# shivendrra/shredword

Measured on AMD Instinct MI355X. Metric: encoded MB/s (input bytes) + Mtokens/s at 32k merges, 1/2/4/8 MI355X vs CPU ref, higher is better.
Workload: dtype int32

## Files before the change

shredword_amd/csrc/encode.hip:

```cpp
#include <hip/hip_runtime.h>

#include <algorithm>
#include <cstdio>
#include <cstring>
#include <string>
#include <vector>

#include "encoder.h"
#include "kernels.h"
#include "long_split.h"
#include "pairtable.h"
#include "presplit_kernel.h"
#include "split_classify.h"
#include "specials_find.h"
#include "test_options.h"

using namespace sw;

static thread_local std::string g_err;
int32_t sw::set_error(int32_t code, const std::string& msg) {
  g_err = msg;
  return code;
}

// ... 559 lines not shown
    }
    SpFind f;
    f.bytes = d_bytes; f.n_bytes = n_bytes; f.str_off = d_str_off; f.n_str = n_str;
    f.tile_slo = h->ws.d_tile_slo; f.n_tiles = n_tiles;
    f.cbits = h->d_spf; f.chosen = h->d_spf + 64 * n_tiles;
    f.tcand = h->d_spf + 128 * n_tiles; f.tcnt = f.tcand + n_tiles;
    f.flag = (unsigned int*)(f.tcnt + n_tiles);
    f.list = h->d_spf_list; f.tcap = tcap;
    int64_t* toff = h->d_spf_off;
    int64_t* toff2 = h->d_spf_off + n_tiles + n_parts;
    int64_t* total2 = toff2 + n_tiles + n_parts;
    const dim3 gw((unsigned)((n_tiles + kWaves - 1) / kWaves)), bw(kThreads);
    HIP_TRY(hipMemsetAsync(f.flag, 0, sizeof(unsigned int), st));
    hipLaunchKernelGGL(k_tile_strings, dim3((unsigned)((n_tiles + 255) / 256)), dim3(256), 0, st, d_str_off, n_str,
                       n_tiles, h->ws.d_tile_slo, nullptr);
    const bool swar = h->spt.n_first <= kSpMaxFirstSwar;
    const size_t lds_tab = sizeof(uint32_t) * (size_t)h->spt.img_words;
    if (swar) hipLaunchKernelGGL(k_sp_find<true>, gw, bw, lds_tab, st, h->spt, f);
    else hipLaunchKernelGGL(k_sp_find<false>, gw, bw, lds_tab, st, h->spt, f);
    HIP_TRY(launch_scan(st, f.tcnt, n_tiles, toff + n_tiles, toff, d_count));
    const dim3 ge((unsigned)((n_tiles + kWaves * kSfEmitTiles - 1) / (kWaves * kSfEmitTiles)));
    hipLaunchKernelGGL(k_sp_emit, ge, bw, 0, st, h->spt, f, (const int64_t*)toff, d_pos, d_len, d_id);
    const dim3 gg(std::min<unsigned>(gw.x, kSfGlobalBlocks));
    if (swar) hipLaunchKernelGGL(k_sp_detect<true>, gg, bw, 0, st, h->spt, f);
    else hipLaunchKernelGGL(k_sp_detect<false>, gg, bw, 0, st, h->spt, f);
    hipLaunchKernelGGL(k_sp_resolve, gg, bw, lds_tab, st, h->spt, f);
    hipLaunchKernelGGL(k_sp_count, gg, bw, 0, st, f);
    HIP_TRY(launch_scan(st, f.tcnt, n_tiles, toff2 + n_tiles, toff2, total2));
    hipLaunchKernelGGL(k_sp_write, gg, bw, 0, st, h->spt, f, (const int64_t*)toff2, d_pos, d_len, d_id);
    hipLaunchKernelGGL(k_sp_fix_count, dim3(1), dim3(64), 0, st, (const unsigned int*)f.flag, (const int64_t*)total2,
                       d_count);
    HIP_TRY(hipGetLastError());
  }
  HIP_TRY(hipEventRecord(h->ws_done, st));
  h->ws_stream = st;
  h->ws_pending = true;
  return SW_OK;
}

namespace {

EncArgs make_args(sw_encoder* h, const uint8_t* d_bytes, int64_t n_bytes, const int64_t* d_str_off, int64_t n_str,
                  const uint64_t* d_chunk_bits, const SpArgs& spa, int64_t* d_out_off, int64_t n_tiles) {
  Workspace& w = h->ws;
  EncArgs a;
  a.bytes = d_bytes; a.n_bytes = n_bytes; a.bits = d_chunk_bits; a.n_words = (n_bytes + 63) / 64;
  a.str_off = d_str_off; a.n_str = n_str; a.table = h->table; a.chunks = h->chunks;
  a.scratch = w.d_scratch; a.res = w.d_res;
  a.tile_slots = w.d_tile_slots; a.tile_nref = w.d_tile_nref; a.rlist = w.d_rlist; a.tile_cnt = w.d_tile_cnt;
  a.dtab = w.d_dtab; a.dedupe = h->dedupe ? 1u : 0u; a.dfp_mask = h->dedupe_fp_mask;
  {
    const uint32_t lmask = (uint32_t)(launch_dd_slots(h, n_bytes) - 1);
    a.dmask = h->dedupe_slots ? std::min<uint32_t>(lmask, (uint32_t)(h->dedupe_slots - 1)) : lmask;
  }
  a.dexact = h->dedupe_exact ? (uint32_t)kDdExactMax : 0u;
  a.dres = w.d_dres;
  a.dcnt = w.d_dcnt;
  a.dd_full = w.d_ddfull;
  a.llist = w.d_llist; a.l_count = w.d_lcount;
  a.big_count = w.d_big; a.big_list = w.d_big + 1;
  a.out_off = d_out_off; a.tile_slo = w.d_tile_slo;
  a.n_tiles = n_tiles; a.qtmp = w.d_res; a.bcnt = w.d_bcnt; a.boff = w.d_boff; a.q_total = w.d_qtotal;
  a.queue = w.d_queue; a.stamps = w.d_stamps;
  a.inv = h->d_inv; a.n_inv = h->n_inv; a.ids16 = h->ids16 ? 1u : 0u;
  a.lstart = w.lp.wstart; a.llen = w.lp.wlen; a.n_long = &w.lp.ctl[kLcWave]; a.lcap = w.lp.lcap;
  a.sp = spa;
  const unsigned long long prev_merges = h->h_ddfull ? __atomic_load_n(&h->h_ddfull[2], __ATOMIC_RELAXED) : 0ULL;
  a.staged_heads = (h->staged_heads == 1 || (h->staged_heads == 0 && h->dedupe && prev_merges > kStagedMinMerges)) ? 1u : 0u;
  return a;
}

template <bool kSp>
hipError_t launch_classify_pair(sw_encoder* h, hipStream_t st, const EncArgs& a, const PbArgs* pg, int pattern,
                                hipEvent_t c0, hipEvent_t c1) {
  const dim3 gc((unsigned)((a.n_tiles + kWaves - 1) / kWaves)), gr(kRedoGrid), b(kThreads);
  unsigned int* count = h->ws.d_redo;
  int64_t* tiles = (int64_t*)(count + 2);
  hipError_t e = c0 ? hipEventRecord(c0, st) : hipSuccess;
  if (e != hipSuccess) return e;
  if (pg) {
    const RedoList redo{count, tiles};
    const uint32_t* edge = h->ws.d_edge;
    uint32_t* pbits = (uint32_t*)h->ws.d_pbits.get();
    hipLaunchKernelGGL(k_split_classify<kSp>, gc, b, 0, st, a, *pg, pattern, edge, pbits, redo);
    if (c1 && (e = hipEventRecord(c1, st)) != hipSuccess) return e;
    hipLaunchKernelGGL(k_split_redo<kSp>, gr, b, 0, st, a, *pg, pattern, edge, pbits, redo);
  } else {
    hipLaunchKernelGGL(k_classify<kSp>, gc, b, 0, st, a, count, tiles);
    if (c1 && (e = hipEventRecord(c1, st)) != hipSuccess) return e;
    hipLaunchKernelGGL(k_classify_big<kSp>, gr, b, 0, st, a, (const unsigned int*)count, (const int64_t*)tiles);
  }
  return hipGetLastError();
}

int32_t launch_classify(sw_encoder* h, hipStream_t st, const EncArgs& a, int32_t pattern, bool fused) {
  const int64_t n_tiles = a.n_tiles;
  const size_t dtab_bytes = sizeof(uint64_t) * kDdWords * ((size_t)a.dmask + 1);
  const int64_t edge_threads = (n_tiles + 1 + 255) / 256 * 256;
  const bool clr_in_edges = fused && dtab_bytes % 16 == 0 && (int64_t)(dtab_bytes / 16) <= 16 * edge_threads;
  if (h->dedupe && !clr_in_edges) HIP_TRY(hipMemsetAsync(h->ws.d_dtab, 0, dtab_bytes, st));
  hipEvent_t c0 = nullptr, c1 = nullptr;
  if (h->timing) HIP_TRY(h->ev_cls.next(&c0, &c1));
  const PbArgs pg{a.bytes, a.n_bytes, a.str_off, a.n_str, a.tile_slo, a.sp};
  if (fused)
    hipLaunchKernelGGL(k_edges, dim3((unsigned)((n_tiles + 1 + 255) / 256)), dim3(256), 0, st, pg, n_tiles, (int)pattern,
                       h->ws.d_edge.get(), h->ws.d_redo.get(), h->dedupe && clr_in_edges ? (uint4*)h->ws.d_dtab.get() : nullptr,
                       (int64_t)(dtab_bytes / 16));
  else
    HIP_TRY(hipMemsetAsync(h->ws.d_redo, 0, sizeof(unsigned int), st));
  HIP_TRY(a.sp.n > 0 ? launch_classify_pair<true>(h, st, a, fused ? &pg : nullptr, (int)pattern, c0, c1)
                     : launch_classify_pair<false>(h, st, a, fused ? &pg : nullptr, (int)pattern, c0, c1));
  if (c1) ++h->ev_cls.used;
  return SW_OK;
}

template <bool kWide, bool k16, bool kWF>
void launch_merge_buckets(const EncArgs& a, const hipStream_t (&ms)[4]) {
  const dim3 pg(2048), pb(kThreads);
  hipLaunchKernelGGL((k_merge_bucket<kWide, k16, 32, kWF>), pg, pb, 0, ms[0], a, 8, 9);
  hipLaunchKernelGGL((k_merge_bucket<kWide, k16, 16, kWF>), pg, pb, 0, ms[1], a, 5, 7);
  hipLaunchKernelGGL((k_merge_bucket<kWide, k16, 8, kWF>), pg, pb, 0, ms[2], a, 3, 4);
  hipLaunchKernelGGL((k_merge_bucket<kWide, k16, 4, kWF>), pg, pb, 0, ms[1], a, 0, 2);
}

template <bool kWide, bool k16, bool kWF>
int32_t launch_merges_as(sw_encoder* h, hipStream_t st, const EncArgs& a) {
  const int64_t n_tiles = a.n_tiles;
  const bool split = h->split_ok && h->long_split;
  hipStream_t ms[4] = {st, st, st, st};
  if (h->merge_fork) {
    for (int k = 0; k < 2; ++k) {
      HIP_TRY(h->s_fork[k].ensure());
      HIP_TRY(h->ev_join[k].ensure());
    }
    HIP_TRY(h->ev_fork.ensure());
    HIP_TRY(h->ev_fork_long.ensure());
    HIP_TRY(hipEventRecord(h->ev_fork_long, st));
    HIP_TRY(hipStreamWaitEvent(h->s_fork[1], h->ev_fork_long, 0));
    ms[1] = h->s_fork[0];
    ms[3] = h->s_fork[1];
  }
  HIP_TRY((launch_long<kWide, k16>(h, ms[3], a, split, 1)));
  HIP_TRY(launch_scan(st, h->ws.d_bcnt, kNumBuckets * n_tiles, h->ws.d_part, h->ws.d_boff, h->ws.d_qtotal));
  hipLaunchKernelGGL(k_scatter, dim3((unsigned)((n_tiles + 15) / 16)), dim3(kThreads), 0, st, a);
  if (h->merge_fork) {
    HIP_TRY(hipEventRecord(h->ev_fork, st));
    for (int k = 0; k < 2; ++k) HIP_TRY(hipStreamWaitEvent(h->s_fork[k], h->ev_fork, 0));
  }
  HIP_TRY((launch_long<kWide, k16>(h, ms[3], a, split, 2)));
  launch_merge_buckets<kWide, k16, kWF>(a, ms);
  if (h->merge_fork) {
    for (int k = 0; k < 2; ++k) {
      HIP_TRY(hipEventRecord(h->ev_join[k], h->s_fork[k]));
      HIP_TRY(hipStreamWaitEvent(st, h->ev_join[k], 0));
    }
  }
  HIP_TRY(hipGetLastError());
  return SW_OK;
}

int32_t launch_merges(sw_encoder* h, hipStream_t st, const EncArgs& a) {
  if (h->table.wide) return launch_merges_as<true, false, false>(h, st, a);
  if (h->ids16 && h->split_ok) return launch_merges_as<false, true, true>(h, st, a);
  if (h->ids16) return launch_merges_as<false, true, false>(h, st, a);
  return launch_merges_as<false, false, false>(h, st, a);
}

// ... 190 lines not shown
```

shredword_amd/csrc/kernels.h:

```cpp
#pragma once
#include <hip/hip_runtime.h>

#include <cstdint>
#include <type_traits>

#include "args.h"
#include "chunktable.h"
#include "table.h"

namespace sw {

constexpr int kThreads = 256;
constexpr int kWaves = kThreads / 64;
__device__ __forceinline__ int wave_in_block() {
  return (int)(threadIdx.x >> 6);
}
__device__ __forceinline__ int64_t tile_end(int64_t t0, int64_t n_bytes) {
  return (int64_t)min((int32_t)t0 + (int32_t)kTile, (int32_t)n_bytes);
}
__device__ __forceinline__ int wave_in_block_s() {
  return __builtin_amdgcn_readfirstlane((int)(threadIdx.x >> 6));
}
constexpr int kShort = 32;
constexpr int kWin = kTile + 64;
// ... 602 lines not shown
      if (prev_taken) M &= ~1ULL;
      uint64_t T = M;
      if (p0 == p1) {
        const uint64_t E = 0x5555555555555555ULL;
        const uint64_t S = M & ~(M << 1);
        const uint64_t runs_even = M & ~(M + (S & E));
        T = (runs_even & E) | (M & ~runs_even & ~E);
      }
      const uint64_t consumed = (T << 1) | (prev_taken ? 1ULL : 0ULL);
      const uint64_t keep = __ballot(valid) & ~consumed;
      const bool take = (T >> lane) & 1ULL;
      const bool next_take = lane < 63 ? ((T >> (lane + 1)) & 1ULL) : true;
      const int64_t pos = w + __popcll(keep & lt_mask);
      wave_sync_mem();
      if ((keep >> lane) & 1ULL) {
        id[pos] = take ? nv : e;
        rk[pos] = (take || next_take) ? RECOMP : er;
      }
      w += __popcll(keep);
      prev_taken = (T >> 63) & 1ULL;
    }
    n = w;
    wave_sync_mem();
  }
  return n;
}

struct SpArgs {
  const int64_t* pos;
  const int32_t* len;
  const int32_t* id;
  int64_t n;
  const int64_t* tile_sp;
  const int64_t* tile_spw;
};

struct EncArgs {
  const uint8_t* bytes;
  int64_t n_bytes;
  const uint64_t* bits;
  int64_t n_words;
  const int64_t* str_off;
  int64_t n_str;
  DevTable table;
  DevChunkTable chunks;
  int32_t* scratch;
  uint32_t* res;
  uint32_t* tile_cnt;
  uint32_t* tile_slots;
  uint32_t* tile_nref;
  uint32_t* rlist;
  int64_t* out_off;
  const int64_t* tile_slo;
  int64_t n_tiles;
  uint32_t* qtmp;
  uint32_t* bcnt;
  const int64_t* boff;
  const int64_t* q_total;
  uint64_t* queue;
  uint64_t* dtab;
  uint32_t dmask;
  uint32_t dfp_mask;
  uint32_t dedupe;
  uint32_t dexact;
  uint4* dres;
  uint8_t* dcnt;
  unsigned long long* dd_full;
  uint64_t* llist;
  unsigned long long* l_count;
  unsigned long long* stamps;
  const uint2* inv;
  uint32_t n_inv;
  const uint32_t* lstart;
  const uint32_t* llen;
  const int64_t* n_long;
  int64_t lcap;
  uint32_t* big_list;
  uint32_t* big_count;
  uint32_t ids16;
  uint32_t staged_heads;
  SpArgs sp;
};

#ifdef SW_STAMPS
#define SW_STAMP(k)                                                                 \
  do {                                                                              \
    if (threadIdx.x == 0) {                                                         \
      const unsigned long long now_ = __builtin_readcyclecounter();                 \
      atomicAdd(&a.stamps[(k) * 64 + (blockIdx.x & 63)], now_ - stamp_prev_);       \
      stamp_prev_ = now_;                                                           \
    }                                                                               \
  } while (0)
#define SW_STAMP_INIT unsigned long long stamp_prev_ = __builtin_readcyclecounter()
#define SW_COUNT(k, v)                                                              \
  do {                                                                              \
    if (threadIdx.x == 0) atomicAdd(&a.stamps[(k) * 64 + (blockIdx.x & 63)], (unsigned long long)(v)); \
  } while (0)
#else
#define SW_COUNT(k, v) do {} while (0)
#define SW_STAMP(k) do {} while (0)
#define SW_STAMP_INIT do {} while (0)
#endif


constexpr uint64_t kDdExact = 1ULL << 63;
struct DdOut {
  int kind;
  uint32_t v;
};

__device__ __forceinline__ DdOut dedupe_claim(const EncArgs& a, const SW_AS_GLOBAL uint32_t* words, int64_t last_word, int64_t mis,
                                              int64_t start, int n, const uint32_t (&u)[kShort / 4]) {
  const int nw = (n + 3) >> 2;
  uint32_t h = 0x9E3779B9u ^ ((uint32_t)n << 24);
#pragma unroll
  for (int q = 0; q < kShort / 4; ++q) {
    if (!__ballot(q < nw)) break;
    if (q < nw) {
      h = (h ^ u[q]) * 0x85EBCA77u;
      h ^= h >> 13;
    }
  }
  const uint32_t h2 = (h ^ (h >> 16)) * 0x7FEB352Du;
  const bool exact = n <= (int)a.dexact;
  const uint64_t lo7 = (uint64_t)u[0] | ((uint64_t)(u[1] & 0xFFFFFFu) << 32);
  const uint64_t tag = exact ? (lo7 | ((uint64_t)n << 56) | kDdExact)
                             : ((uint64_t)((h2 >> 6) & a.dfp_mask & 0x3FFFFFFu) << 37 | (uint64_t)n << 31);
  const uint64_t mine = exact ? tag : (tag | (uint64_t)start);
  const uint32_t grp = h & a.dmask & ~(kDdGroup - 1);
  for (int j = 0; j < (int)kDdGroup; ++j) {
    const uint32_t idx = grp | ((h2 + j) & (kDdGroup - 1));
    unsigned long long* p = (unsigned long long*)a.dtab + (size_t)kDdWords * idx;
    uint64_t cur = *p;
    if (cur == 0) {
      cur = atomicCAS(p, 0ULL, (unsigned long long)mine);
      if (cur == 0) return DdOut{1, idx};
    }
    if (exact) {
      if (cur == mine) return DdOut{2, idx};
      continue;
    }
    if ((cur & ~0x7FFFFFFFULL) != tag) continue;
    const int64_t other = (int64_t)(cur & 0x7FFFFFFFULL);
    const int64_t g = other + mis, w0 = g >> 2;
    const uint32_t sh = (uint32_t)(g & 3);
    bool same = true;
    if ((((uintptr_t)words & 15) == 0) && ((g + n - 1) >> 4) <= ((last_word + 1) >> 2) - 1) {
      const uint4* q16 = (const uint4*)words;
      const int64_t b0 = g >> 4;
      const int span = (int)(g & 15) + n;
      const uint4 x0 = q16[b0];
      const uint4 x1 = span > 16 ? q16[b0 + 1] : make_uint4(0, 0, 0, 0);
      const uint4 x2 = span > 32 ? q16[b0 + 2] : make_uint4(0, 0, 0, 0);
      const uint32_t W[12] = {x0.x, x0.y, x0.z, x0.w, x1.x, x1.y, x1.z, x1.w, x2.x, x2.y, x2.z, x2.w};
      const int k = (int)(w0 & 3);
      uint32_t R[kShort / 4 + 1];
#pragma unroll
      for (int i = 0; i <= kShort / 4; ++i) R[i] = k == 0 ? W[i] : k == 1 ? W[i + 1] : k == 2 ? W[i + 2] : W[i + 3];
#pragma unroll
      for (int q = 0; q < kShort / 4; ++q) {
        if (q < nw) {
          const int keep = n - 4 * q;
          const uint32_t x = __builtin_amdgcn_alignbyte(R[q + 1], R[q], sh);
          const uint32_t m = keep >= 4 ? ~0u : ((1u << (8 * keep)) - 1u);
          same = same && ((x & m) == u[q]);
        }
// ... 61 lines not shown
  const int64_t s_first = a.tile_slo[tile];
  const int64_t sp_lo = kSp ? a.sp.tile_sp[tile] : 0, sp_hi = kSp ? a.sp.tile_sp[tile + 1] : 0;

  static_assert(kTile == 64 * 32, "a tile's bits are 64 lanes x 32");
  uint32_t myhalf;
  {
    const uint32_t lo = (uint32_t)__shfl((int)(uint32_t)bw, lane >> 1, 64);
    const uint32_t hi = (uint32_t)__shfl((int)(uint32_t)(bw >> 32), lane >> 1, 64);
    myhalf = (lane & 1) ? hi : lo;
    const int64_t lim = t1 - (t0 + 32 * lane);
    if (lim <= 0) myhalf = 0;
    else if (lim < 32) myhalf &= (1u << lim) - 1u;
  }
  int64_t last_end = a.n_bytes;
  {
    uint64_t hw = 0;
    const int64_t bit0 = t0 + 64 * (int64_t)lane;
    if (lane < kTileWords && bit0 + 64 > t1) {
      hw = bw;
      if (bit0 < t1) hw &= ~0ULL << (t1 - bit0);
    }
    const uint64_t has = __ballot(hw != 0);
    if (has) {
      const int src = __ffsll((long long)has) - 1;
      const int64_t q = t0 + 64 * (int64_t)src + __ffsll((long long)__shfl(hw, src, 64)) - 1;
      last_end = min(q, a.n_bytes);
    } else if (__ballot(myhalf != 0)) {
      const int64_t q = next_set_bit(a.bits, a.n_words, t0 + 64 * kTileWords, a.n_bytes);
      last_end = min(q, a.n_bytes);
    }
  }
  classify_chunks<kSp>(a, tile, s_b32, s_cstart, s_qbuf, myhalf, (int)(last_end - t0), s_first, sp_lo, sp_hi, cap,
                       ov_count, ov_tiles);
}

template <bool kSp>
__device__ __forceinline__ void classify_chunks(const EncArgs& a, int64_t tile, const uint32_t* s_b32,
                                                uint16_t* s_cstart, uint16_t* s_qbuf, uint32_t myhalf, int rel_end,
                                                int64_t s_first, int64_t sp_lo, int64_t sp_hi, int cap,
                                                unsigned int* ov_count, int64_t* ov_tiles) {
  SW_STAMP_INIT;
  const int lane = threadIdx.x & 63;
  const uint64_t lt_mask = (lane == 0) ? 0ULL : (~0ULL >> (64 - lane));
  const int64_t t0 = tile * kTile;
  const int64_t t1 = tile_end(t0, a.n_bytes);
  const uint32_t cnt = (uint32_t)__popc(myhalf);
  const uint32_t incl = wave_incl_scan(cnt, lane);
  const int C = (int)lane_value(incl, 63);
  if (C > cap) {
    if (lane == 0) ov_tiles[atomicAdd(ov_count, 1u)] = tile;
    return;
  }
  {
    uint32_t x = myhalf;
    uint32_t k = incl - cnt;
    while (x) {
      s_cstart[k++] = (uint16_t)(32 * lane + __ffs(x) - 1);
      x &= x - 1;
    }
  }
  wave_sync_mem();
  if (kSp) {
    if (sp_lo < 0) {
      sp_lo = a.sp.tile_sp[tile];
      sp_hi = a.sp.tile_sp[tile + 1];
    }
    for (int64_t j = sp_lo + lane; j < sp_hi; j += 64) {
      const int p = (int)(a.sp.pos[j] - t0);
      int lo = 0, hi = C;
      while (lo < hi) {
        const int m = (lo + hi) >> 1;
        if ((int)(s_cstart[m] & kCsPos) < p) lo = m + 1; else hi = m;
      }
      if (lo < C && (int)s_cstart[lo] == p) {
        s_cstart[lo] = (uint16_t)(p | kCsSpecial);
        SW_STNT(&a.scratch[t0 + lo], (int32_t)a.sp.id[j]);
      }
    }
    wave_sync_mem();
  }
  SW_STAMP(0);

  int32_t* dst = a.scratch + t0;
  const int rounds = (C + 63) >> 6;
#ifdef SW_DIAG_NO_LOOKUP
  const bool use_table = false;
#else
  const bool use_table = a.chunks.enabled != 0;
#endif
  const int64_t mis = (int64_t)((uintptr_t)a.bytes & 3);
  const SW_AS_GLOBAL uint32_t* gwords = (const SW_AS_GLOBAL uint32_t*)((uintptr_t)a.bytes - mis);
  const int64_t last_word = (mis + a.n_bytes - 1) >> 2;
  uint32_t bcount = 0;
  int nq = 0;
  int nown = 0;
  int nref = 0;
  for (int r0 = 0; r0 < rounds || nq > 0; r0 += kLookRounds) {
    if (r0 < rounds) {
      uint32_t tok[kLookRounds];
      if (use_table) {
        table_lookups<kLookRounds, kSp>(a.chunks, s_b32, s_cstart, C, rel_end, r0, lane, tok);
      } else {
#pragma unroll
        for (int u = 0; u < kLookRounds; ++u) {
          const int k = ((r0 + u) << 6) + lane;
          const bool valid = k < C;
          const uint32_t cs = valid ? s_cstart[k] : 0u;
          const int ls = (int)(cs & kCsPos);
          const int end = (k + 1 < C) ? (int)(s_cstart[k + 1] & kCsPos) : rel_end;
          tok[u] = (kSp && (cs & kCsSpecial)) ? kSpDone
                   : (valid && end - ls == 1) ? (s_b32[ls >> 2] >> (8 * (ls & 3))) & 0xFFu
#ifdef SW_DIAG_NO_LOOKUP
                   : (valid && end - ls <= kShort) ? 0u
#endif
                   : kInf;
        }
      }
#pragma unroll
      for (int u = 0; u < kLookRounds; ++u) {
        const int k = ((r0 + u) << 6) + lane;
        const bool valid = k < C;
        const bool queued = valid && tok[u] == kInf;
        if (valid && !queued && (!kSp || tok[u] != kSpDone)) SW_STNT(&dst[k], (int32_t)tok[u]);
        const uint64_t mq = __ballot(queued);
        if (queued) s_qbuf[nq + __popcll(mq & lt_mask)] = (uint16_t)k;
        nq += __popcll(mq);
      }
    }
    while (nq >= 64 || (r0 + kLookRounds >= rounds && nq > 0)) {
      wave_sync_mem();
      SW_STAMP(1);
      const bool act = lane < nq;
      const int k = act ? s_qbuf[lane] : 0;
      uint16_t rest[kQBuf / 64 - 1];
#pragma unroll
      for (int q = 1; q < kQBuf / 64; ++q) rest[q - 1] = (64 * q + lane < nq) ? s_qbuf[64 * q + lane] : 0;
#pragma unroll
      for (int q = 1; q < kQBuf / 64; ++q)
        if (64 * q + lane < nq) s_qbuf[64 * (q - 1) + lane] = rest[q - 1];
      nq = nq > 64 ? nq - 64 : 0;
      const int ls = act ? (int)(s_cstart[k] & kCsPos) : 0;
      const int end = (k + 1 < C) ? (int)(s_cstart[k + 1] & kCsPos) : rel_end;
      const int len = act ? end - ls : 0;
      DdOut dd{0, 0};
      if (act && a.dedupe && len <= kShort) {
        uint32_t u[kShort / 4];
        window_words(s_b32, ls, min(len, 16), *(uint32_t(*)[4])u);
        if (len > 16) window_words(s_b32, ls + 16, len - 16, *(uint32_t(*)[4])(u + 4));
        else
#pragma unroll
          for (int q = 4; q < kShort / 4; ++q) u[q] = 0;
        dd = dedupe_claim(a, gwords, last_word, mis, t0 + ls, len, u);
      }
      const uint32_t did = dd.kind ? dd.v : kNoDid;
      if (act) {
        const int64_t own = t0 + ls;
        dst[k] = dd.kind ? slot_dref(did) : slot_ref(own);
        SW_STNT2(&a.rlist[t0 + nref + lane], dd.kind ? (kRlDense | did) : (uint32_t)own);
      }
      nref += (int)__popcll(__ballot(act));
      const bool longc = act && len > kShort;
      const uint64_t lm = __ballot(longc);
      if (lm) {
        unsigned long long lb = 0;
        if (lane == 0) lb = atomicAdd(a.l_count, (unsigned long long)__popcll(lm));
        lb = lane_value64(lb, 0);
        if (longc)
          a.llist[lb + __popcll(lm & lt_mask)] =
              ((uint64_t)(t0 + ls) << 32) | (len < (int)kNoDid ? (uint32_t)len : kNoDid);
      }
      const bool queued = act && dd.kind != 2 && !longc;
      const int b = queued ? bucket_of(len) : 15;
      uint64_t pend = __ballot(queued);
      if (queued) {
        const int64_t qi = t0 + nown + __popcll(pend & lt_mask);
        SW_STNT2(&a.qtmp[qi], (uint32_t)ls | ((uint32_t)k << kTileBits) | ((uint32_t)len << (2 * kTileBits)));
        SW_STNT2(&a.qtmp[qi + kTile / 2], did);
      }
      nown += __popcll(pend);
      while (pend) {
        const int bb = (int)lane_value((uint32_t)b, __ffsll((long long)pend) - 1);
        const uint64_t m = __ballot(b == bb);
        if (lane == bb) bcount += (uint32_t)__popcll(m);
        pend &= ~m;
      }
      wave_sync_mem();
      SW_STAMP(7);
    }
  }
  SW_STAMP(1);

  if (lane < kNumBuckets) a.bcnt[(int64_t)lane * a.n_tiles + tile] = bcount;
  if (lane == 0) {
    a.tile_slots[tile] = (uint32_t)C;
    a.tile_nref[tile] = (uint32_t)nref;
  }
  SW_STAMP(2);

  (void)s_first;
  const int64_t s_first_now = a.tile_slo[tile];
  for (int64_t s = s_first_now + lane; s < a.n_str; s += 64) {
    const int64_t p = a.str_off[s];
    if (p >= t1) break;
    int lo = 0, hi = C;
    const int lp = (int)(p - t0);
    while (lo < hi) {
      const int m = (lo + hi) >> 1;
      if ((int)(s_cstart[m] & kCsPos) < lp) lo = m + 1; else hi = m;
    }
    a.out_off[s] = (int64_t)lo;
  }
  SW_STAMP(3);
  wave_sync_mem();
}

template <bool kSp>
__global__ void __launch_bounds__(kThreads) __attribute__((amdgpu_waves_per_eu(7, 7))) k_classify(EncArgs a, unsigned int* ov_count, int64_t* ov_tiles) {
  __shared__ __attribute__((aligned(16))) uint32_t s_b32_all[kWaves][kWinWords];
  __shared__ uint16_t s_cs_all[kWaves][kClsCsCap + 1];
  __shared__ uint16_t s_qb_all[kWaves][kQBuf];
  const int wv = wave_in_block_s();
  const int64_t tile = (int64_t)blockIdx.x * kWaves + wv;
  if (tile < a.n_tiles)
    classify_tile<kSp>(a, tile, s_b32_all[wv], s_cs_all[wv], s_qb_all[wv], kClsCsCap, ov_count, ov_tiles);
}

template <bool kSp>
__global__ void __launch_bounds__(kThreads) k_classify_big(EncArgs a, const unsigned int* ov_count, const int64_t* ov_tiles) {
  __shared__ __attribute__((aligned(16))) uint32_t s_b32_all[kWaves][kWinWords];
  __shared__ uint16_t s_cs_all[kWaves][kTile + 1];
  __shared__ uint16_t s_qb_all[kWaves][kQBuf];
  const int wv = wave_in_block_s();
  const int64_t n = (int64_t)__hip_atomic_load(ov_count, __ATOMIC_RELAXED, __HIP_MEMORY_SCOPE_AGENT);
  for (int64_t i = (int64_t)blockIdx.x * kWaves + wv; i < n; i += (int64_t)gridDim.x * kWaves) {
    const int64_t tile = __hip_atomic_load(&ov_tiles[i], __ATOMIC_RELAXED, __HIP_MEMORY_SCOPE_AGENT);
    classify_tile<kSp>(a, tile, s_b32_all[wv], s_cs_all[wv], s_qb_all[wv], kTile + 1, nullptr, nullptr);
  }
}

template <int kG>
__device__ __forceinline__ void scatter_round(const EncArgs& a, int64_t t0, bool act, uint32_t e, uint32_t did,
                                              int64_t& dst) {
  const int lane = threadIdx.x & 63, g = lane / kG;
  const uint64_t lt_mask = (lane == 0) ? 0ULL : (~0ULL >> (64 - lane));
  const uint64_t gmask = (kG == 64 ? ~0ULL : ((1ULL << kG) - 1ULL)) << (kG * g);
  const uint32_t ns = e >> (2 * kTileBits);
  const int b = act ? (ns ? bucket_of(ns) : kLongBucket) : 15;
  if (a.dedupe) {
    const uint64_t full = __ballot(act && ns != 0 && did == kNoDid);
    if (full && lane == 0) atomicAdd(a.dd_full, (unsigned long long)__popcll(full));
  }
  int64_t d = 0;
  uint64_t pend = __ballot(act);
  while (pend) {
    const uint64_t pg = pend & gmask;
    const int bb = pg ? __shfl(b, __ffsll((long long)pg) - 1, 64) : -1;
    const bool mine = act && b == bb && ((pend >> lane) & 1);
    const uint64_t m = __ballot(mine);
    const int64_t db = __shfl(dst, kG * g + (bb < 0 ? 0 : bb), 64);
    if (mine) d = db + __popcll(m & gmask & lt_mask);
    if (lane - kG * g == bb) dst += __popcll(m & gmask);
    pend &= ~m;
  }
  if (act) {
    const uint64_t start = (uint64_t)(t0 + (e & (kTile - 1)));
    a.queue[d] = (start << 33) | ((uint64_t)ns << 27) | did;
  }
}

__global__ void __launch_bounds__(kThreads) k_scatter(EncArgs a) {
  constexpr int kG = 16;
  const int lane = threadIdx.x & 63, g = lane >> 4, gl = lane & (kG - 1);
  const int64_t tb = ((int64_t)blockIdx.x * kWaves + wave_in_block()) * (64 / kG);
  const int64_t t = tb + g;
  const bool tile_ok = t < a.n_tiles;
  uint32_t c = 0;
  int64_t dst = 0;
  if (tile_ok && gl < kNumBuckets) {
    c = a.bcnt[(int64_t)gl * a.n_tiles + t];
    dst = a.boff[(int64_t)gl * a.n_tiles + t];
  }
  uint32_t n = c;
#pragma unroll
  for (int off = 1; off < kG; off <<= 1) n += __shfl_xor(n, off, 64);
  {
    const bool act = tile_ok && n <= (uint32_t)kG && (uint32_t)gl < n;
    const uint32_t e = act ? SW_LDNT2(&a.qtmp[t * kTile + gl]) : 0u;
// ... 1034 lines not shown
```

shredword_amd/csrc/presplit_bits.h:

```cpp
#pragma once
#include <cstdint>

#include "presplit_match.h"

namespace sw {
namespace psb {

#define SW_PSB_FI __attribute__((always_inline))

constexpr int kChunk = 32;

constexpr uint32_t kLane7 = 0x80808080u, kLow7 = 0x7F7F7F7Fu, kLane0 = 0x01010101u;

SW_HD inline uint32_t in7(uint32_t x7, uint32_t lo, uint32_t hi) {
  return (x7 + kLane0 * (0x80 - lo)) & ~(x7 + kLane0 * (0x7F - hi)) & kLane7;
}

struct Masks {
  uint32_t L, N, C, P, H, A, X, K1, K2;
};

SW_HD inline uint32_t mm4(uint32_t x) { return ((x & 0x80808080u) * 0x00204081u) >> 28; }

SW_HD inline uint64_t rev64(uint64_t x) {
#if defined(__HIP_DEVICE_COMPILE__)
  return __builtin_bitreverse64(x);
#else
  x = ((x >> 1) & 0x5555555555555555ULL) | ((x & 0x5555555555555555ULL) << 1);
  x = ((x >> 2) & 0x3333333333333333ULL) | ((x & 0x3333333333333333ULL) << 2);
  x = ((x >> 4) & 0x0F0F0F0F0F0F0F0FULL) | ((x & 0x0F0F0F0F0F0F0F0FULL) << 4);
  x = ((x >> 8) & 0x00FF00FF00FF00FFULL) | ((x & 0x00FF00FF00FF00FFULL) << 8);
  x = ((x >> 16) & 0x0000FFFF0000FFFFULL) | ((x & 0x0000FFFF0000FFFFULL) << 16);
  return (x >> 32) | (x << 32);
#endif
}

SW_HD inline uint64_t fill_up(uint64_t Y, uint64_t R) { return ((R + (Y & R)) ^ R) & R; }
SW_HD inline uint64_t fill_down(uint64_t Y, uint64_t R) { return rev64(fill_up(rev64(Y), rev64(R))); }

struct RegBytes {
  uint32_t w[10];
  SW_HD uint32_t word(int i) const { return w[i]; }
  SW_HD uint32_t at4(int k) const {
    uint32_t lo_w = w[0], hi_w = w[1];
#pragma unroll
    for (int q = 1; q < 10; ++q) {
      lo_w = (k >> 2) == q ? w[q] : lo_w;
      hi_w = (k >> 2) == q ? (q + 1 < 10 ? w[q + 1] : 0u) : hi_w;
    }
    return (uint32_t)((((uint64_t)hi_w << 32) | lo_w) >> (8 * (k & 3)));
  }
};

SW_HD inline uint32_t perm_b32(uint32_t hi, uint32_t lo, uint32_t sel) {
#if defined(__HIP_DEVICE_COMPILE__)
  return __builtin_amdgcn_perm(hi, lo, sel);
#else
  const uint64_t v = ((uint64_t)hi << 32) | lo;
  uint32_t r = 0;
  for (int k = 0; k < 4; ++k) {
    const uint32_t q = (sel >> (8 * k)) & 0xFFu;
    const uint32_t byte = q < 8 ? (uint32_t)(v >> (8 * q)) & 0xFFu : q == 12 ? 0u : q >= 13 ? 0xFFu : 0u;
    r |= byte << (8 * k);
  }
  return r;
#endif
}

SW_HD inline uint32_t ascii_class4(uint32_t x) {
  const uint32_t lo = x & 0x07070707u;
  const uint32_t pa = perm_b32(0xD8C8C8C8u, 0xC8C8C868u, lo);
  const uint32_t pb = perm_b32(0x80808482u, 0x828CCAC8u, lo);
  const uint32_t nm8 = perm_b32(0xFFFFFFFFu, 0u, (x & 0x08080808u) | 0x04040404u);
  const uint32_t tlo = (nm8 & pa) | (~nm8 & pb);
  const uint32_t thi = perm_b32(0x08800880u, 0x40300006u, (x >> 4) & 0x07070707u);
  return tlo & thi;
}
SW_HD inline uint32_t mm8(uint32_t x) { return ((x & 0x88888888u) * 0x00204081u) >> 24; }

SW_HD inline int fast_class(uint32_t cp) {
  auto in = [](uint32_t x, uint32_t lo, uint32_t hi) -> uint32_t { return x - lo <= hi - lo ? 1u : 0u; };
  const uint32_t L = (in(cp, 0xC0, 0x2C1) & (cp != 0xD7 ? 1u : 0u) & (cp != 0xF7 ? 1u : 0u)) | in(cp, 0x391, 0x3A1) |
                     in(cp, 0x3A3, 0x3F5) | in(cp, 0x3F7, 0x481) | in(cp, 0x48A, 0x52F) | in(cp, 0x3041, 0x3096) |
                     in(cp, 0x30A1, 0x30FA) | in(cp, 0x3400, 0x4DBF) | in(cp, 0x4E00, 0xA48C) | in(cp, 0xAC00, 0xD7A3) |
                     in(cp, 0x20000, 0x2A6DF);
  return L ? kL : in(cp, 0x1F10D, 0x1FBEF) ? kOther : -1;
}

template <class Cls, class Bytes>
SW_HD inline Masks classify(const Bytes& by, uint64_t ss, const Cls& cls, bool cl) {
  uint32_t L = 0, N = 0, C = 0, P = 0, H = 0, A = 0;
#pragma unroll
  for (int i = 1; i < 9; ++i) {
    const uint32_t t = ascii_class4(by.word(i));
    const int s = 4 * (i - 1);
    const uint32_t l = mm8(t), nc = mm8(t << 1), ph = mm8(t << 2);
    L |= ((l >> 4) | (l & 15u)) << s;
    N |= (nc >> 4) << s;
    C |= (nc & 15u) << s;
    P |= (ph >> 4) << s;
    H |= (ph & 15u) << s;
    A |= mm4(t << 3) << s;
  }
  uint64_t X = 0;
  uint64_t hi40 = 0, ct40 = 0;
#pragma unroll
  for (int i = 0; i < 10; ++i) hi40 |= (uint64_t)mm4(by.word(i)) << (4 * i);
  {
    const uint32_t asc = ~(uint32_t)(hi40 >> 4);
    L &= asc; N &= asc; C &= asc; P &= asc; H &= asc; A &= asc;
  }
  if (hi40) {
#pragma unroll
    for (int i = 0; i < 10; ++i) {
      const uint32_t x = by.word(i), h7 = (x ^ kLane7) & kLow7;
      ct40 |= (uint64_t)mm4(in7(h7, 0x00, 0x3F) & x & kLane7) << (4 * i);
    }
    auto lead = [&](int k, uint64_t* tail_out) -> uint32_t {
      const uint32_t b4 = by.at4(k), c0 = b4 & 0xFFu, c1 = (b4 >> 8) & 0xFFu;
      const int n = c0 >= 0xF0 ? 4 : c0 >= 0xE0 ? 3 : 2;
      const uint64_t tail = ((1ULL << (n - 1)) - 1ULL) << (k + 1);
      bool ok = (ct40 & tail) == tail && (ss & tail) == 0 && c0 >= 0xC2 && c0 <= 0xF4;
      ok = ok && !(c0 == 0xE0 && c1 < 0xA0) && !(c0 == 0xED && c1 > 0x9F) && !(c0 == 0xF0 && c1 < 0x90) &&
           !(c0 == 0xF4 && c1 > 0x8F);
      *tail_out = ok ? tail : 0ULL;
      if (!ok || k < 4) return kInvalidCp;
      uint32_t v = c0 & (n == 2 ? 0x1Fu : n == 3 ? 0x0Fu : 0x07u);
      for (int q = 1; q < n; ++q) v = (v << 6) | ((b4 >> (8 * q)) & 0x3Fu);
      return v;
    };
    auto apply = [&](int k, uint32_t v, int c) {
      const uint32_t bit = v == kInvalidCp ? 0u : 1u << (k - 4);
      L |= c == kL ? bit : 0u;
      N |= c == kN ? bit : 0u;
      H |= c == kS ? bit : 0u;
    };
    for (uint64_t m = hi40 & ~ct40 & 0xFFFFFFFFFULL; m; m &= m - 1) {
      const int k = __builtin_ctzll(m);
      uint64_t t;
      const uint32_t v = lead(k, &t);
      X |= t;
      if (v != kInvalidCp) {
        int c = fast_class(v);
#if defined(SW_DIAG_NO_UCD)
        if (c < 0) c = kOther;
#endif
        if (c < 0) c = cls(v);
        apply(k, v, c);
      }
    }
  }
  uint32_t K1 = 0, K2 = 0;
  for (uint32_t m = A; m; m &= m - 1) {
    const int a = __builtin_ctz(m), k = a + 5;
    if ((ss >> k) & 1) continue;
    const uint32_t b4 = by.at4(k), c1 = b4 & 0xFFu, c2 = (b4 >> 8) & 0xFFu;
    const uint32_t l1 = cl && c1 >= 'A' && c1 <= 'Z' ? c1 | 0x20u : c1, l2 = cl && c2 >= 'A' && c2 <= 'Z' ? c2 | 0x20u : c2;
    const bool two_ok = !((ss >> (k + 1)) & 1);
    if (l1 == 's' || l1 == 'd' || l1 == 'm' || l1 == 't' || (cl && c1 == 0xC5 && c2 == 0xBF && two_ok)) {
      K1 |= 1u << a;
    } else if (two_ok && ((l1 == 'l' && l2 == 'l') || (l1 == 'v' && l2 == 'e') || (l1 == 'r' && l2 == 'e'))) {
      K2 |= 1u << a;
    }
  }
  Masks r;
  r.L = L; r.N = N; r.C = C; r.P = P; r.H = H; r.A = A; r.X = (uint32_t)(X >> 4); r.K1 = K1; r.K2 = K2;
  return r;
}

struct Carry {
  int digit = -1;
  int cro = -1;
  int hasc = -1;
};
enum : uint32_t { kNeedDigit = 1, kNeedCro = 2, kNeedHasc = 4 };

SW_HD inline uint64_t window(uint32_t before, uint32_t mine, uint32_t after) {
  return (uint64_t)(before >> 16) | ((uint64_t)mine << 16) | ((uint64_t)after << 48);
}

SW_HD inline uint32_t rules(const Masks& m0, const Masks& m1, const Masks& m2, uint64_t ssw, bool cl, const Carry& cy,
                            uint32_t* need) {
  const uint64_t X = window(m0.X, m1.X, m2.X);
  const uint64_t L = window(m0.L, m1.L, m2.L), N = window(m0.N, m1.N, m2.N), C = window(m0.C, m1.C, m2.C);
  const uint64_t P = window(m0.P, m1.P, m2.P), H = window(m0.H, m1.H, m2.H), A = window(m0.A, m1.A, m2.A);
  const uint64_t K1 = window(m0.K1, m1.K1, m2.K1), K2 = window(m0.K2, m1.K2, m2.K2);
  const uint64_t LEAD = ~X, WS = C | P | H, O = LEAD & ~(L | N | WS), PH_ = P | H;
  constexpr uint64_t kPay = 0x0000FFFFFFFF0000ULL;
  auto F = [&](uint64_t M) -> uint64_t { return ((X + (M << 1)) & ~X) & ~ssw; };
  auto B = [&](uint64_t M) -> uint64_t {
    const uint64_t y = rev64(((M & LEAD & ~ssw) >> 1)), rx = rev64(X);
    return rev64((rx + y) & ~rx);
  };
  const uint64_t PL = F(L), PN = F(N), PO = F(O), PP = F(P), PC = F(C), PWS = F(WS);
  const uint64_t first = LEAD & (~LEAD + 1);
  *need = 0;
  uint64_t st;
  const uint64_t NNW = B(LEAD & ~WS);
  if (cl) {
    const uint64_t OST = O & ~PO & ~PP;
// ... 116 lines not shown
```

shredword_amd/csrc/split_classify.h:

```cpp
#pragma once
#include <hip/hip_runtime.h>

#include <cstdint>

#include "kernels.h"
#include "presplit_bits.h"
#include "presplit_kernel.h"

namespace sw {

constexpr int kEdgeWords = 10;

__device__ __forceinline__ uint32_t ss32_hint(const int64_t* str_off, int64_t n_str, int64_t n_bytes,
                                              const int64_t* tile_slo, int64_t n_tiles, int64_t p) {
  if (p > n_bytes) return 0u;
  int64_t lo = 0, hi = 0;
  if (p > 0) {
    const int64_t t = p >> kTileBits;
    lo = t < n_tiles ? tile_slo[t] : n_str;
    hi = t + 1 < n_tiles ? tile_slo[t + 1] : n_str;
  }
  while (lo < hi) {
    const int64_t m = (lo + hi) >> 1;
    if (str_off[m] < p) lo = m + 1; else hi = m;
// ... 280 lines not shown
  const int64_t wb = t0 - kScPre;
  uint32_t rw[10];
  static_assert(kScPre == 32 && kWin == kTile + 64, "block layout of the window");
  const bool fast = ((uintptr_t)a.bytes & 15) == 0 && wb >= 0 && wb + kScPre + kWin <= a.n_bytes;
  if (fast) {
    const u32x4* src = (const u32x4*)(a.bytes + wb);
    const u32x4 x0 = SW_LDNT(src + 2 + 2 * lane), x1 = SW_LDNT(src + 3 + 2 * lane);
    const bool ex = lane < 5 || lane == 63;
    const int eb = lane == 0 ? 1 : lane == 1 ? 0 : lane == 63 ? 130 : 129 + lane;
    u32x4 xe = u32x4{0, 0, 0, 0};
    if (ex) xe = SW_LDNT(src + eb);
    *(uint4*)(s_win + 4 * (2 + 2 * lane)) = make_uint4(x0[0], x0[1], x0[2], x0[3]);
    *(uint4*)(s_win + 4 * (3 + 2 * lane)) = make_uint4(x1[0], x1[1], x1[2], x1[3]);
    if (ex) *(uint4*)(s_win + 4 * eb) = make_uint4(xe[0], xe[1], xe[2], xe[3]);
    rw[1] = x0[0]; rw[2] = x0[1]; rw[3] = x0[2]; rw[4] = x0[3];
    rw[5] = x1[0]; rw[6] = x1[1]; rw[7] = x1[2]; rw[8] = x1[3];
    const uint32_t up = (uint32_t)__builtin_amdgcn_update_dpp(0, (int)rw[8], 0x13C, 0xF, 0xF, false);
    const uint32_t dn = (uint32_t)__builtin_amdgcn_update_dpp(0, (int)rw[1], 0x134, 0xF, 0xF, false);
    rw[0] = lane == 0 ? xe[3] : up;
    rw[9] = lane == 63 ? xe[0] : dn;
  } else {
    for (int i = lane; i < (kScPre + kWin) / 4; i += 64) {
      const int64_t p = wb + 4 * (int64_t)i;
      uint32_t v = 0;
      for (int k = 0; k < 4; ++k) v |= (p + k >= 0 && p + k < a.n_bytes ? (uint32_t)a.bytes[p + k] : 0u) << (8 * k);
      s_win[i] = v;
    }
  }
  if (lane < 8) s_win[(kScPre + kWin) / 4 + lane] = 0;
  if (!fast) {
    wave_sync_mem();
#pragma unroll
    for (int i = 0; i < 10; ++i) rw[i] = s_win[kScPre / 4 - 1 + 8 * lane + i];
  }
  const uint32_t r0 = edge[9 * stride + tile], r_next = edge[9 * stride + tile + 1];
  const int64_t s_first = a.tile_slo[tile];
  ScMasks& sm = sh->pre;
  if (lane < 9) sm.m[lane][65] = edge[lane * stride + tile + 1];
  else if (lane < 18) sm.m[lane - 9][0] = 0u;
  for (int i = lane; i < kScSsWords; i += 64) sm.ss[i] = 0;
  wave_sync_mem();
  {
    const int64_t first = tile > 0 ? a.tile_slo[tile - 1] : 0;
    for (int64_t i0 = first; i0 <= a.n_str; i0 += 64) {
      const int64_t i = i0 + lane;
      int64_t r = (int64_t)kScSsWords * 32;
      if (i <= a.n_str) r = a.str_off[i] - (t0 - kScSsPre);
      if (r >= 0 && r < (int64_t)kScSsWords * 32) atomicOr(&sm.ss[r >> 5], 1u << (r & 31));
      if (__ballot(r < (int64_t)kScSsWords * 32) != ~0ULL) break;
    }
  }
  constexpr bool has_sp = kSp;
  if (has_sp) {
    sm.in[lane] = 0u;
    wave_sync_mem();
    const int64_t w0 = t0 - kScSsPre, w1 = w0 + (int64_t)kScSsWords * 32;
    const int64_t nsp = a.sp.tile_sp[a.n_tiles];
    const int64_t j_first = a.sp.tile_spw[tile];
    for (int64_t j0 = j_first; j0 < nsp; j0 += 64) {
      const int64_t j = j0 + lane;
      int64_t pa = w1, pe = w1;
      if (j < nsp) {
        pa = a.sp.pos[j];
        pe = pa + a.sp.len[j];
      }
      if (pa < w1) {
        if (pa >= w0) atomicOr(&sm.ss[(pa - w0) >> 5], 1u << ((pa - w0) & 31));
        if (pe >= w0 && pe < w1) atomicOr(&sm.ss[(pe - w0) >> 5], 1u << ((pe - w0) & 31));
        for (int64_t q = max(pa + 1, t0); q < min(pe, t0 + (int64_t)kTile);) {
          const int64_t qe = min(min(pe, t0 + (int64_t)kTile), ((q - t0) | 31) + 1 + t0);
          const int sh = (int)((q - t0) & 31), nb = (int)(qe - q);
          atomicOr(&sm.in[(q - t0) >> 5], (nb >= 32 ? ~0u : ((1u << nb) - 1u)) << sh);
          q = qe;
        }
      }
      if (__ballot(pa < w1) != ~0ULL) break;
    }
  }
  wave_sync_mem();
#ifdef SW_STAMPS
  __builtin_amdgcn_s_waitcnt(0);
  SW_STAMP(12);
#endif
  const FSrc src{GSrc{g, a.n_tiles, n_chunks, cl}, &sm, c0, t0, n_chunks};
  uint32_t r = 0;
  bool unresolved = false;
  if (pattern == 2) {
    if (c < n_chunks) r = src.ss(c);
  } else {
    {
      psb::Masks m1{};
      if (c < n_chunks) {
        const MixBytes by{rw, s_win + (kScPre / 4 - 1) + 8 * lane};
        const int64_t p = 32 * c;
        const uint64_t s = (uint64_t)src.ss_at(p - 4) | ((uint64_t)(src.ss_at(p + 28) & 0xFFu) << 32);
        m1 = psb::classify(by, s, UcdClass{}, cl);
      }
      const int k = lane + 1;
      sm.m[0][k] = m1.L; sm.m[1][k] = m1.N; sm.m[2][k] = m1.C; sm.m[3][k] = m1.P; sm.m[4][k] = m1.H;
      sm.m[5][k] = m1.A; sm.m[6][k] = m1.X; sm.m[7][k] = m1.K1; sm.m[8][k] = m1.K2;
    }
    wave_sync_mem();
    SW_STAMP(13);
    auto col = [&](int k) {
      return psb::Masks{sm.m[0][k], sm.m[1][k], sm.m[2][k], sm.m[3][k], sm.m[4][k], sm.m[5][k], sm.m[6][k], sm.m[7][k], sm.m[8][k]};
    };
    if (c < n_chunks) {
      const int64_t p = 32 * c;
      const uint64_t ssw = (uint64_t)src.ss_at(p - 16) | ((uint64_t)src.ss_at(p + 16) << 32);
      uint32_t need = 0;
      r = psb::rules(col(lane), col(lane + 1), col(lane + 2), ssw, cl, psb::Carry{}, &need);
      if (lane == 0) {
        r = r0;
        need = 0;
      }
      if (need) {
        if constexpr (kRedo) {
          const psb::Carry cy = psb::carries(src, c, need);
          asm volatile("" ::: "memory");
          r = psb::rules(col(lane), col(lane + 1), col(lane + 2), ssw, cl, cy, &need);
        } else {
          bool hit = false;
          const LSrc ls{&sm, c0, t0, n_chunks, &hit};
          const psb::Carry cy = psb::carries(ls, c, need);
          asm volatile("" ::: "memory");
          if (hit) unresolved = true;
          else r = psb::rules(col(lane), col(lane + 1), col(lane + 2), ssw, cl, cy, &need);
        }
      }
    }
  }
  if (c < n_chunks) {
    if (has_sp && lane > 0) r &= ~sm.in[lane];
    if (32 * c + 32 > a.n_bytes) r &= (1u << (a.n_bytes - 32 * c)) - 1u;
  }
  if constexpr (!kRedo) {
    constexpr int kCap = (int)(sizeof(sh->cstart) / sizeof(uint16_t)) - 2;
    bool over = false;
    if constexpr (kCap < kTile) over = wave_sum((uint32_t)__popc(c < n_chunks ? r : 0u), lane) > (uint32_t)kCap;
    if (__ballot(unresolved) || over) {
      if (lane == 0) redo.tiles[atomicAdd(redo.count, 1u)] = tile;
      return;
    }
  }
  if (c < n_chunks) {
    bits32[c] = r;
    if (c == n_chunks - 1 && (c & 1) == 0) bits32[c + 1] = 0;
  }
  SW_STAMP(14);
  int rel_end;
  if (t1 >= a.n_bytes) rel_end = (int)(a.n_bytes - t0);
  else if (r_next != 0) rel_end = kTile + __builtin_ctz(r_next);
  else if (a.n_bytes <= t1 + 32) rel_end = (int)(a.n_bytes - t0);
  else rel_end = kRelEndLong;
  wave_sync_mem();
    classify_chunks<kSp>(a, tile, s_win + kScPre / 4, sh->cstart, s_qbuf, r, rel_end, s_first, -1, -1);
}

template <bool kSp>
__global__ void __launch_bounds__(kThreads) __attribute__((amdgpu_waves_per_eu(7, 7)))
k_split_classify(EncArgs a, PbArgs g, int pattern, const uint32_t* edge, uint32_t* bits32, RedoList redo) {
  __shared__ __attribute__((aligned(16))) uint32_t s_win_all[kWaves][kScWinWords];
  __shared__ ScSharedT<kScCsCap> s_sh_all[kWaves];
  __shared__ uint16_t s_qb_all[kWaves][kQBuf];
  const int wv = wave_in_block_s();
  const int64_t tile = (int64_t)blockIdx.x * kWaves + wv;
  if (tile < a.n_tiles)
    split_classify_tile<kSp, false>(a, g, pattern, edge, bits32, tile, s_win_all[wv], &s_sh_all[wv], s_qb_all[wv],
                                    redo);
}

constexpr int kRedoGrid = 256;
template <bool kSp>
__global__ void __launch_bounds__(kThreads) k_split_redo(EncArgs a, PbArgs g, int pattern, const uint32_t* edge,
                                                         uint32_t* bits32, RedoList redo) {
  __shared__ __attribute__((aligned(16))) uint32_t s_win_all[kWaves][kScWinWords];
  __shared__ ScShared s_sh_all[kWaves];
  __shared__ uint16_t s_qb_all[kWaves][kQBuf];
  const int wv = wave_in_block_s();
  const int64_t n = (int64_t)__hip_atomic_load(redo.count, __ATOMIC_RELAXED, __HIP_MEMORY_SCOPE_AGENT);
  for (int64_t i = (int64_t)blockIdx.x * kWaves + wv; i < n; i += (int64_t)gridDim.x * kWaves) {
    const int64_t tile = __hip_atomic_load(&redo.tiles[i], __ATOMIC_RELAXED, __HIP_MEMORY_SCOPE_AGENT);
    split_classify_tile<kSp, true>(a, g, pattern, edge, bits32, tile, s_win_all[wv], &s_sh_all[wv], s_qb_all[wv],
                                   redo);
    wave_sync_mem();
  }
}

}
```

Before: 266,200.

## Rewrite byte-class bit extraction with perm/dot4 transpose and read kernargs by reference

```diff
diff --git a/shredword_amd/csrc/encode.hip b/shredword_amd/csrc/encode.hip
--- a/shredword_amd/csrc/encode.hip
+++ b/shredword_amd/csrc/encode.hip
@@ -665,7 +665,7 @@
     const RedoList redo{count, tiles};
     const uint32_t* edge = h->ws.d_edge;
     uint32_t* pbits = (uint32_t*)h->ws.d_pbits.get();
-    hipLaunchKernelGGL(k_split_classify<kSp>, gc, b, 0, st, a, *pg, pattern, edge, pbits, redo);
+    hipLaunchKernelGGL(k_split_classify<kSp>, gc, b, 0, st, ScArgs{a, *pg, pattern, edge, pbits, redo});
     if (c1 && (e = hipEventRecord(c1, st)) != hipSuccess) return e;
     hipLaunchKernelGGL(k_split_redo<kSp>, gr, b, 0, st, a, *pg, pattern, edge, pbits, redo);
   } else {
diff --git a/shredword_amd/csrc/kernels.h b/shredword_amd/csrc/kernels.h
--- a/shredword_amd/csrc/kernels.h
+++ b/shredword_amd/csrc/kernels.h
@@ -708,6 +708,11 @@
   SpArgs sp;
 };
 
+#ifndef SW_DIAG_PHASES
+#define SW_DIAG_PHASES 0
+#endif
+constexpr int kDiagPhases = SW_DIAG_PHASES;
+
 #ifdef SW_STAMPS
 #define SW_STAMP(k)                                                                 \
   do {                                                                              \
@@ -935,7 +940,8 @@
   SW_STAMP(0);
 
   int32_t* dst = a.scratch + t0;
-  const int rounds = (C + 63) >> 6;
+  const int C_out = kDiagPhases == 4 ? 0 : C;
+  const int rounds = (C_out + 63) >> 6;
 #ifdef SW_DIAG_NO_LOOKUP
   const bool use_table = false;
 #else
@@ -973,6 +979,7 @@
       for (int u = 0; u < kLookRounds; ++u) {
         const int k = ((r0 + u) << 6) + lane;
         const bool valid = k < C;
+        if (kDiagPhases == 5 && tok[u] == kInf) tok[u] = 0u;
         const bool queued = valid && tok[u] == kInf;
         if (valid && !queued && (!kSp || tok[u] != kSpDone)) SW_STNT(&dst[k], (int32_t)tok[u]);
         const uint64_t mq = __ballot(queued);
@@ -1045,7 +1052,7 @@
 
   if (lane < kNumBuckets) a.bcnt[(int64_t)lane * a.n_tiles + tile] = bcount;
   if (lane == 0) {
-    a.tile_slots[tile] = (uint32_t)C;
+    a.tile_slots[tile] = (uint32_t)C_out;
     a.tile_nref[tile] = (uint32_t)nref;
   }
   SW_STAMP(2);
@@ -1055,7 +1062,7 @@
   for (int64_t s = s_first_now + lane; s < a.n_str; s += 64) {
     const int64_t p = a.str_off[s];
     if (p >= t1) break;
-    int lo = 0, hi = C;
+    int lo = 0, hi = C_out;
     const int lp = (int)(p - t0);
     while (lo < hi) {
       const int m = (lo + hi) >> 1;
diff --git a/shredword_amd/csrc/presplit_bits.h b/shredword_amd/csrc/presplit_bits.h
--- a/shredword_amd/csrc/presplit_bits.h
+++ b/shredword_amd/csrc/presplit_bits.h
@@ -20,7 +20,25 @@
   uint32_t L, N, C, P, H, A, X, K1, K2;
 };
 
-SW_HD inline uint32_t mm4(uint32_t x) { return ((x & 0x80808080u) * 0x00204081u) >> 28; }
+SW_HD inline uint32_t dot4_u8(uint32_t a, uint32_t b, uint32_t c) {
+#if defined(__HIP_DEVICE_COMPILE__)
+  return __builtin_amdgcn_udot4(a, b, c, false);
+#else
+  for (int k = 0; k < 4; ++k) c += ((a >> (8 * k)) & 0xFFu) * ((b >> (8 * k)) & 0xFFu);
+  return c;
+#endif
+}
+
+template <int B>
+SW_HD inline uint32_t bits8_raw(uint32_t lo, uint32_t hi) {
+  return dot4_u8(hi & (kLane0 << B), 0x80402010u, dot4_u8(lo & (kLane0 << B), 0x08040201u, 0u));
+}
+template <int B, class W>
+SW_HD inline uint32_t bits32(const W& w) {
+  const uint32_t lo = bits8_raw<B>(w(0), w(1)) | (bits8_raw<B>(w(2), w(3)) << 8);
+  const uint32_t hi = bits8_raw<B>(w(4), w(5)) | (bits8_raw<B>(w(6), w(7)) << 8);
+  return (lo >> B) | ((hi >> B) << 16);
+}
 
 SW_HD inline uint64_t rev64(uint64_t x) {
 #if defined(__HIP_DEVICE_COMPILE__)
@@ -76,7 +94,33 @@
   const uint32_t thi = perm_b32(0x08800880u, 0x40300006u, (x >> 4) & 0x07070707u);
   return tlo & thi;
 }
-SW_HD inline uint32_t mm8(uint32_t x) { return ((x & 0x88888888u) * 0x00204081u) >> 24; }
+
+SW_HD inline void bit_planes32(uint32_t (&w)[8]) {
+  uint32_t u[8];
+#pragma unroll
+  for (int g = 0; g < 2; ++g) {
+    const uint32_t p0 = perm_b32(w[g + 2], w[g], 0x05010400u), p1 = perm_b32(w[g + 2], w[g], 0x07030602u);
+    const uint32_t q0 = perm_b32(w[g + 6], w[g + 4], 0x05010400u), q1 = perm_b32(w[g + 6], w[g + 4], 0x07030602u);
+    u[4 * g + 0] = perm_b32(q0, p0, 0x05040100u);
+    u[4 * g + 1] = perm_b32(q0, p0, 0x07060302u);
+    u[4 * g + 2] = perm_b32(q1, p1, 0x05040100u);
+    u[4 * g + 3] = perm_b32(q1, p1, 0x07060302u);
+  }
+  auto swap_blocks = [&](int s, uint32_t low) {
+#pragma unroll
+    for (int r = 0; r < 8; ++r) {
+      if (r & s) continue;
+      const uint32_t a = u[r], b = u[r + s];
+      u[r] = (a & low) | ((b << s) & ~low);
+      u[r + s] = ((a >> s) & low) | (b & ~low);
+    }
+  };
+  swap_blocks(4, 0x0F0F0F0Fu);
+  swap_blocks(2, 0x33333333u);
+  swap_blocks(1, 0x55555555u);
+#pragma unroll
+  for (int r = 0; r < 8; ++r) w[r] = u[r];
+}
 
 SW_HD inline int fast_class(uint32_t cp) {
   auto in = [](uint32_t x, uint32_t lo, uint32_t hi) -> uint32_t { return x - lo <= hi - lo ? 1u : 0u; };
@@ -89,33 +133,31 @@
 
 template <class Cls, class Bytes>
 SW_HD inline Masks classify(const Bytes& by, uint64_t ss, const Cls& cls, bool cl) {
-  uint32_t L = 0, N = 0, C = 0, P = 0, H = 0, A = 0;
-#pragma unroll
-  for (int i = 1; i < 9; ++i) {
-    const uint32_t t = ascii_class4(by.word(i));
-    const int s = 4 * (i - 1);
-    const uint32_t l = mm8(t), nc = mm8(t << 1), ph = mm8(t << 2);
-    L |= ((l >> 4) | (l & 15u)) << s;
-    N |= (nc >> 4) << s;
-    C |= (nc & 15u) << s;
-    P |= (ph >> 4) << s;
-    H |= (ph & 15u) << s;
-    A |= mm4(t << 3) << s;
-  }
+  uint32_t t[8];
+#pragma unroll
+  for (int i = 0; i < 8; ++i) {
+    const uint32_t x = by.word(i + 1);
+    t[i] = ascii_class4(x) | ((x >> 7) & kLane0);
+  }
+  bit_planes32(t);
+  uint32_t L = t[7] | t[3], N = t[6], C = t[2], P = t[5], H = t[1], A = t[4];
   uint64_t X = 0;
-  uint64_t hi40 = 0, ct40 = 0;
-#pragma unroll
-  for (int i = 0; i < 10; ++i) hi40 |= (uint64_t)mm4(by.word(i)) << (4 * i);
+  uint64_t ct40 = 0;
+  auto ends8 = [&](uint32_t u0, uint32_t u9) -> uint64_t {
+    const uint32_t e = bits8_raw<7>(u0, u9) >> 7;
+    return (uint64_t)(e & 15u) | ((uint64_t)(e >> 4) << 36);
+  };
+  const uint64_t hi40 = ((uint64_t)t[0] << 4) | ends8(by.word(0), by.word(9));
   {
     const uint32_t asc = ~(uint32_t)(hi40 >> 4);
     L &= asc; N &= asc; C &= asc; P &= asc; H &= asc; A &= asc;
   }
   if (hi40) {
-#pragma unroll
-    for (int i = 0; i < 10; ++i) {
-      const uint32_t x = by.word(i), h7 = (x ^ kLane7) & kLow7;
-      ct40 |= (uint64_t)mm4(in7(h7, 0x00, 0x3F) & x & kLane7) << (4 * i);
-    }
+    auto ct4 = [&](int i) -> uint32_t {
+      const uint32_t x = by.word(i);
+      return in7(x & kLow7, 0x00, 0x3F) & x;
+    };
+    ct40 = ((uint64_t)bits32<7>([&](int i) -> uint32_t { return ct4(i + 1); }) << 4) | ends8(ct4(0), ct4(9));
     auto lead = [&](int k, uint64_t* tail_out) -> uint32_t {
       const uint32_t b4 = by.at4(k), c0 = b4 & 0xFFu, c1 = (b4 >> 8) & 0xFFu;
       const int n = c0 >= 0xF0 ? 4 : c0 >= 0xE0 ? 3 : 2;
diff --git a/shredword_amd/csrc/split_classify.h b/shredword_amd/csrc/split_classify.h
--- a/shredword_amd/csrc/split_classify.h
+++ b/shredword_amd/csrc/split_classify.h
@@ -386,18 +386,22 @@
   __builtin_amdgcn_s_waitcnt(0);
   SW_STAMP(12);
 #endif
-  const FSrc src{GSrc{g, a.n_tiles, n_chunks, cl}, &sm, c0, t0, n_chunks};
+  auto ss_rel = [&](int d) -> uint32_t {
+    const int r = kScSsPre + 32 * lane + d, wi = r >> 5;
+    return (uint32_t)(((uint64_t)sm.ss[wi] | ((uint64_t)sm.ss[wi + 1] << 32)) >> (r & 31));
+  };
+  static_assert(kScSsPre + 32 * 63 + 96 + 32 <= kScSsWords * 32 && kScSsPre >= 16, "ss_rel stays inside the staged words");
   uint32_t r = 0;
   bool unresolved = false;
-  if (pattern == 2) {
-    if (c < n_chunks) r = src.ss(c);
+  if (kDiagPhases == 1) {
+  } else if (pattern == 2) {
+    if (c < n_chunks) r = ss_rel(0);
   } else {
     {
       psb::Masks m1{};
       if (c < n_chunks) {
         const MixBytes by{rw, s_win + (kScPre / 4 - 1) + 8 * lane};
-        const int64_t p = 32 * c;
-        const uint64_t s = (uint64_t)src.ss_at(p - 4) | ((uint64_t)(src.ss_at(p + 28) & 0xFFu) << 32);
+        const uint64_t s = (uint64_t)ss_rel(-4) | ((uint64_t)(ss_rel(28) & 0xFFu) << 32);
         m1 = psb::classify(by, s, UcdClass{}, cl);
       }
       const int k = lane + 1;
@@ -409,9 +413,8 @@
     auto col = [&](int k) {
       return psb::Masks{sm.m[0][k], sm.m[1][k], sm.m[2][k], sm.m[3][k], sm.m[4][k], sm.m[5][k], sm.m[6][k], sm.m[7][k], sm.m[8][k]};
     };
-    if (c < n_chunks) {
-      const int64_t p = 32 * c;
-      const uint64_t ssw = (uint64_t)src.ss_at(p - 16) | ((uint64_t)src.ss_at(p + 16) << 32);
+    if (kDiagPhases != 2 && c < n_chunks) {
+      const uint64_t ssw = (uint64_t)ss_rel(-16) | ((uint64_t)ss_rel(16) << 32);
       uint32_t need = 0;
       r = psb::rules(col(lane), col(lane + 1), col(lane + 2), ssw, cl, psb::Carry{}, &need);
       if (lane == 0) {
@@ -420,6 +423,7 @@
       }
       if (need) {
         if constexpr (kRedo) {
+          const FSrc src{GSrc{g, a.n_tiles, n_chunks, cl}, &sm, c0, t0, n_chunks};
           const psb::Carry cy = psb::carries(src, c, need);
           asm volatile("" ::: "memory");
           r = psb::rules(col(lane), col(lane + 1), col(lane + 2), ssw, cl, cy, &need);
@@ -458,20 +462,31 @@
   else if (a.n_bytes <= t1 + 32) rel_end = (int)(a.n_bytes - t0);
   else rel_end = kRelEndLong;
   wave_sync_mem();
-    classify_chunks<kSp>(a, tile, s_win + kScPre / 4, sh->cstart, s_qbuf, r, rel_end, s_first, -1, -1);
-}
+    classify_chunks<kSp>(a, tile, s_win + kScPre / 4, sh->cstart, s_qbuf,
+                         kDiagPhases >= 1 && kDiagPhases <= 3 ? 0u : r, rel_end, s_first, -1, -1);
+}
+
+struct ScArgs {
+  EncArgs a;
+  PbArgs g;
+  int pattern;
+  const uint32_t* edge;
+  uint32_t* bits32;
+  RedoList redo;
+};
 
 template <bool kSp>
-__global__ void __launch_bounds__(kThreads) __attribute__((amdgpu_waves_per_eu(7, 7)))
-k_split_classify(EncArgs a, PbArgs g, int pattern, const uint32_t* edge, uint32_t* bits32, RedoList redo) {
+__global__ void __launch_bounds__(kThreads) __attribute__((amdgpu_waves_per_eu(7, 7))) k_split_classify(ScArgs by_value) {
   __shared__ __attribute__((aligned(16))) uint32_t s_win_all[kWaves][kScWinWords];
   __shared__ ScSharedT<kScCsCap> s_sh_all[kWaves];
   __shared__ uint16_t s_qb_all[kWaves][kQBuf];
+  (void)by_value;
+  const ScArgs& k = *(const ScArgs*)__builtin_amdgcn_kernarg_segment_ptr();
   const int wv = wave_in_block_s();
   const int64_t tile = (int64_t)blockIdx.x * kWaves + wv;
-  if (tile < a.n_tiles)
-    split_classify_tile<kSp, false>(a, g, pattern, edge, bits32, tile, s_win_all[wv], &s_sh_all[wv], s_qb_all[wv],
-                                    redo);
+  if (tile < k.a.n_tiles)
+    split_classify_tile<kSp, false>(k.a, k.g, k.pattern, k.edge, k.bits32, tile, s_win_all[wv], &s_sh_all[wv],
+                                    s_qb_all[wv], k.redo);
 }
 
 constexpr int kRedoGrid = 256;
```

Result: faster. 290,000, median of 6 (+9.0%).
